# hkchengrex/Cutie

Measured on NVIDIA H100. Metric: frames/sec @480p 3-obj, higher is better.
Workload: dtype f32

## Files before the change

cutie_b200/csrc/conv_tc.cu:

```cuda
#include "common.cuh"
#include "tc_ptx.cuh"

namespace cutie {

namespace {

constexpr int CV_M = 128;
constexpr int CV_KC = 32;
constexpr int CV_A_STAGES = 3;
constexpr int CV_THREADS = 384;
constexpr int CV_WARPS = CV_THREADS / 32;
constexpr int CV_PROD = 128;
constexpr int CV3_ROWS = 248;
constexpr int CV1_ROWS = 128;
constexpr int CV_STAGING = 65 * 1024;

__host__ __device__ constexpr int cv_row_bytes(bool f16) { return f16 ? 64 : 128; }
__host__ __device__ constexpr int cv_planes(bool f16) { return f16 ? 1 : 2; }
__host__ __device__ constexpr int cv_a_bytes(bool f16) { return cv_planes(f16) * CV_M * cv_row_bytes(f16); }
__host__ __device__ constexpr int cv_x_bytes(int ks, bool f16) {
  const int operands = (ks == 3 ? 2 * CV3_ROWS : 4 * CV1_ROWS) * cv_planes(f16) * cv_row_bytes(f16);
  return operands > CV_STAGING ? operands : CV_STAGING;
}

struct ConvTail {
  unsigned long long a_full[2][CV_A_STAGES], a_empty[2][CV_A_STAGES], x_full[4], x_empty[4];
  int last[2];
};
constexpr int cv_smem(int ks, bool f16) { return cv_x_bytes(ks, f16) + CV_A_STAGES * cv_a_bytes(f16) + (int)sizeof(ConvTail) + 64; }

struct ConvTcParams {
  const float* x;
  const unsigned char* wimg;
  const float* bias;
  const float* z;
  float* y;
  long long xs_n, xs_c, xs_p;
  long long ys_n, ys_c, ys_p;
  long long zs_n, zs_c, zs_p;
  int Cin, Cout, H, W;
  int Hi, Wi, stride;
  int TH, TW, tiles_x;
  int pitch, xoff;
  int plane_rows;
  int shift[9];
  int N;
  int relu_in, relu_out, x_vec;
  int cl_vec;
  int q;
  int T, tiles, cots;
  int maxslots;
  float* ws;
  int* counters;
};

struct ConvPart {
  int tile, cot, nb;
  int ty0, tx0;
  long long pix0;
  int c0, c1;
  int slot, nslots;
  long long tile_lin;
};

template <int KS, bool F16>
__global__ void __launch_bounds__(CV_THREADS, 1) conv_tc_kernel(const ConvTcParams p) {
  constexpr int XROWS = KS == 3 ? CV3_ROWS : CV1_ROWS;
  constexpr int ROWB = cv_row_bytes(F16);
  constexpr int XPLANE = XROWS * ROWB;
  constexpr int XSTAGE = cv_planes(F16) * XPLANE;
  constexpr int XST = KS == 3 ? 2 : 4;
  constexpr int A_BYTES = cv_a_bytes(F16);
  constexpr int TAPS = KS * KS;
  constexpr int RPT = KS == 3 ? 2 : 1;
  constexpr int DEPTH = KS == 3 ? 1 : 2;
  constexpr int A_HALF = 64 * ROWB;
  extern __shared__ __align__(1024) unsigned char smem[];
  unsigned char* Xs = smem;
  unsigned char* As = smem + cv_x_bytes(KS, F16);
  ConvTail& T = *reinterpret_cast<ConvTail*>(As + CV_A_STAGES * A_BYTES);
  const int tid = threadIdx.x, lane = tid & 31, warp = tid >> 5;
  const int TWp = p.pitch;
  const int C = p.Cin / CV_KC;
  const long long HW = (long long)p.H * p.W;
  const long long U = (long long)p.T * C;
  const long long u0 = (long long)blockIdx.x * p.q, u1 = u0 + p.q < U ? u0 + p.q : U;
  auto make_part = [&](long long ua, long long ub) {
    ConvPart P;
    P.tile_lin = ua / C;
    P.c0 = (int)(ua - P.tile_lin * C);
    P.c1 = P.c0 + (int)(ub - ua);
    const long long first = (P.tile_lin * C) / p.q, last = (P.tile_lin * C + C - 1) / p.q;
    P.slot = (int)(blockIdx.x - first);
    P.nslots = (int)(last - first + 1);
    P.tile = (int)(P.tile_lin % p.tiles);
    const long long rest = P.tile_lin / p.tiles;
    P.cot = (int)(rest % p.cots);
    P.nb = (int)(rest / p.cots);
    P.ty0 = KS == 3 ? (P.tile / p.tiles_x) * p.TH : 0;
    P.tx0 = KS == 3 ? (P.tile % p.tiles_x) * p.TW : 0;
    P.pix0 = (long long)P.tile * p.N;
    return P;
  };
  const long long split_at = (u0 / C + 1) * C < u1 ? (u0 / C + 1) * C : u1;
  const int nparts = split_at < u1 ? 2 : 1;
  const ConvPart part0 = make_part(u0, split_at), part1 = make_part(nparts == 2 ? split_at : u0, u1);
  const bool direct = nparts == 1 && part0.nslots == 1;

  if (tid == 0) {
    for (int G = 0; G < 2; ++G)
      for (int s = 0; s < CV_A_STAGES; ++s) { mbar_init(smem_u32(&T.a_full[G][s]), 1); mbar_init(smem_u32(&T.a_empty[G][s]), 128); }
    for (int s = 0; s < XST; ++s) { mbar_init(smem_u32(&T.x_full[s]), CV_PROD); mbar_init(smem_u32(&T.x_empty[s]), 256); }
    T.last[0] = T.last[1] = 0;
    mbar_init_fence();
  }
  __syncthreads();
  const bool staged_nchw = p.ys_p == 1 && (p.z == nullptr || p.zs_p == 1);
  const bool staged = staged_nchw || p.cl_vec;
  const int LD = p.N | 1;
  auto store_staged_rows = [&](const ConvPart& P, int sw) {
    const float* stage = reinterpret_cast<const float*>(smem);
    if (!staged_nchw) {
      const int co4 = P.cot * CV_M + 4 * lane;
      if (co4 >= p.Cout) return;
      const float4 b4 = p.bias ? __ldg(reinterpret_cast<const float4*>(p.bias + co4)) : make_float4(0.f, 0.f, 0.f, 0.f);
      for (int j = sw; j < p.N; j += CV_WARPS) {
        long long pix;
        bool ok;
        if (KS == 3) {
          const int ty = j / TWp, lx = j - ty * TWp;
          const int gy = P.ty0 + ty, gx = P.tx0 + lx - p.xoff;
          ok = lx >= p.xoff && lx < p.TW + p.xoff && ty < p.TH && gy < p.H && gx < p.W;
          pix = (long long)gy * p.W + gx;
        } else {
          pix = P.pix0 + j;
          ok = pix < HW;
        }
        if (!ok) continue;
        float4 v = *reinterpret_cast<const float4*>(stage + j * CV_M + 4 * lane);
        v.x += b4.x; v.y += b4.y; v.z += b4.z; v.w += b4.w;
        if (p.z) {
          const float4 z4 = __ldg(reinterpret_cast<const float4*>(p.z + (long long)P.nb * p.zs_n + pix * p.zs_p + co4));
          v.x += z4.x; v.y += z4.y; v.z += z4.z; v.w += z4.w;
        }
        if (p.relu_out) v = make_float4(fmaxf(v.x, 0.f), fmaxf(v.y, 0.f), fmaxf(v.z, 0.f), fmaxf(v.w, 0.f));
        *reinterpret_cast<float4*>(p.y + (long long)P.nb * p.ys_n + pix * p.ys_p + co4) = v;
      }
      return;
    }
    const int nseg = CV_M * (KS == 3 ? p.TH : 1);
    for (int seg = sw; seg < nseg; seg += CV_WARPS) {
      const int col = KS == 3 ? seg / p.TH : seg, ty = KS == 3 ? seg - col * p.TH : 0;
      const int co = P.cot * CV_M + col;
      if (co >= p.Cout) continue;
      long long pbase;
      int len, sbase;
      if (KS == 3) {
        const int gy = P.ty0 + ty;
        if (gy >= p.H) continue;
        pbase = (long long)gy * p.W + P.tx0;
        len = p.W - P.tx0 < p.TW ? p.W - P.tx0 : p.TW;
        sbase = col * LD + ty * TWp + p.xoff;
      } else {
        pbase = P.pix0;
        len = HW - P.pix0 < p.N ? (int)(HW - P.pix0) : p.N;
        sbase = col * LD;
      }
      const float b = p.bias ? __ldg(p.bias + co) : 0.f;
      float* yrow = p.y + (long long)P.nb * p.ys_n + (long long)co * p.ys_c + pbase;
      const float* zrow = p.z ? p.z + (long long)P.nb * p.zs_n + (long long)co * p.zs_c + pbase : nullptr;
      for (int i = lane; i < len; i += 32) {
        float val = stage[sbase + i] + b;
        if (zrow) val += __ldg(zrow + i);
        if (p.relu_out) val = fmaxf(val, 0.f);
        yrow[i] = val;
      }
    }
  };

  auto reduce_shares = [&](const ConvPart& P, int sw, bool to_stage) {
    const int co4 = P.cot * CV_M + 4 * lane;
    const float* wst = p.ws + (P.tile_lin * p.maxslots) * (long long)(p.N * CV_M) + 4 * lane;
    float* stage = reinterpret_cast<float*>(smem);
    const bool co_ok = co4 < p.Cout;
    const float4 b4 = (!to_stage && p.bias && co_ok) ? __ldg(reinterpret_cast<const float4*>(p.bias + co4)) : make_float4(0.f, 0.f, 0.f, 0.f);
    for (int j = sw; j < p.N; j += CV_WARPS) {
      long long pix = 0;
      bool ok = true;
      if (!to_stage) {
        if (KS == 3) {
          const int ty = j / TWp, lx = j - ty * TWp;
          const int gy = P.ty0 + ty, gx = P.tx0 + lx - p.xoff;
          ok = lx >= p.xoff && lx < p.TW + p.xoff && ty < p.TH && gy < p.H && gx < p.W;
          pix = (long long)gy * p.W + gx;
        } else {
          pix = P.pix0 + j;
          ok = pix < HW;
        }
        if (!ok || !co_ok) continue;
      }
      float4 v = __ldcg(reinterpret_cast<const float4*>(wst + (long long)j * CV_M));
      for (int k = 1; k < P.nslots; ++k) {
        const float4 t = __ldcg(reinterpret_cast<const float4*>(wst + ((long long)k * p.N + j) * CV_M));
        v.x += t.x; v.y += t.y; v.z += t.z; v.w += t.w;
      }
      if (to_stage) {
        stage[(4 * lane + 0) * LD + j] = v.x; stage[(4 * lane + 1) * LD + j] = v.y;
        stage[(4 * lane + 2) * LD + j] = v.z; stage[(4 * lane + 3) * LD + j] = v.w;
      } else {
        v.x += b4.x; v.y += b4.y; v.z += b4.z; v.w += b4.w;
        if (p.z) {
          const float4 z4 = __ldg(reinterpret_cast<const float4*>(p.z + (long long)P.nb * p.zs_n + pix * p.zs_p + co4));
          v.x += z4.x; v.y += z4.y; v.z += z4.z; v.w += z4.w;
        }
        if (p.relu_out) v = make_float4(fmaxf(v.x, 0.f), fmaxf(v.y, 0.f), fmaxf(v.z, 0.f), fmaxf(v.w, 0.f));
        *reinterpret_cast<float4*>(p.y + (long long)P.nb * p.ys_n + pix * p.ys_p + co4) = v;
      }
    }
  };

  if (warp >= 8) {
    const int pt = tid - 256;
    int xc = 0;
    for (int pi = 0; pi < nparts; ++pi) {
      const ConvPart& P = pi ? part1 : part0;
      const int chunks = P.c1 - P.c0;
      bool valid[RPT];
      const float* xb[RPT];
#pragma unroll
      for (int h = 0; h < RPT; ++h) {
        const int r = pt + CV_PROD * h;
        bool ok = false;
        long long poff = 0;
        if (KS == 3) {
          if (p.stride == 1) {
            const int rows_used = p.N + 2 * TWp + 2;
            if (r >= 1 && r < rows_used) {
              const int q = r - 1, ly = q / TWp, lx = q - ly * TWp;
              const int gy = P.ty0 + ly - 1, gx = P.tx0 + lx - 1;
              ok = ly < p.TH + 2 && gy >= 0 && gy < p.Hi && gx >= 0 && gx < p.Wi;
              poff = (long long)gy * p.Wi + gx;
            }
          } else {
            const int pl = r / p.plane_rows, q = r - pl * p.plane_rows;
            const int lu = q / TWp, lv = q - lu * TWp;
            const int gy = 2 * (P.ty0 - 1 + lu) + (pl >> 1), gx = 2 * (P.tx0 - 1 + lv) + (pl & 1);
            ok = pl < 4 && lu <= p.TH && gy >= 0 && gy < p.Hi && gx >= 0 && gx < p.Wi;
            poff = (long long)gy * p.Wi + gx;
          }
        } else {
          const long long op = P.pix0 + r;
          if (r < p.N && op < HW) {
            const int oy = (int)(op / p.W), ox = (int)(op - (long long)oy * p.W);
            ok = true;
            poff = (long long)(oy * p.stride) * p.Wi + ox * p.stride;
          }
        }
        valid[h] = ok;
        xb[h] = p.x + (long long)P.nb * p.xs_n + poff * p.xs_p + (long long)(P.c0 * CV_KC) * p.xs_c;
      }
      float v[DEPTH][RPT][CV_KC];
      auto load = [&](int c, float (&dst)[RPT][CV_KC]) {
#pragma unroll
        for (int h = 0; h < RPT; ++h) {
          if (p.x_vec) {
#pragma unroll
            for (int k4 = 0; k4 < CV_KC / 4; ++k4) {
              const float4 f = valid[h] ? __ldg(reinterpret_cast<const float4*>(xb[h] + c * CV_KC + 4 * k4)) : make_float4(0.f, 0.f, 0.f, 0.f);
              dst[h][4 * k4] = f.x; dst[h][4 * k4 + 1] = f.y; dst[h][4 * k4 + 2] = f.z; dst[h][4 * k4 + 3] = f.w;
            }
          } else {
#pragma unroll
            for (int i = 0; i < CV_KC; ++i) dst[h][i] = valid[h] ? __ldg(xb[h] + (long long)(c * CV_KC + i) * p.xs_c) : 0.f;
          }
        }
      };
#pragma unroll
      for (int d = 0; d < DEPTH; ++d)
        if (d < chunks) load(d, v[d]);
#pragma unroll 1
      for (int cb = 0; cb < chunks; cb += DEPTH) {
#pragma unroll
        for (int d = 0; d < DEPTH; ++d) {
          const int c = cb + d;
          if (c < chunks) {
            const int s = xc % XST;
            mbar_wait(smem_u32(&T.x_empty[s]), ((xc / XST) & 1) ^ 1);
#pragma unroll
            for (int rh = 0; rh < RPT; ++rh) {
              const int r = pt + CV_PROD * rh;
              if (r >= XROWS) continue;
              const float* src = v[d][rh];
              if (F16) {
                unsigned char* row = Xs + s * XSTAGE + r * ROWB;
#pragma unroll
                for (int k8 = 0; k8 < CV_KC / 8; ++k8) {
                  float f[8];
#pragma unroll
                  for (int i = 0; i < 8; ++i) f[i] = p.relu_in ? fmaxf(src[8 * k8 + i], 0.f) : src[8 * k8 + i];
                  const int off = (k8 ^ ((r >> 1) & 3)) << 4;
                  *reinterpret_cast<uint4*>(row + off) =
                      make_uint4(f16x2_rn(f[0], f[1]), f16x2_rn(f[2], f[3]), f16x2_rn(f[4], f[5]), f16x2_rn(f[6], f[7]));
                }
              } else {
                unsigned char* hi = Xs + s * XSTAGE + r * 128;
                unsigned char* lo = hi + XPLANE;
#pragma unroll
                for (int k4 = 0; k4 < CV_KC / 4; ++k4) {
                  float4 f = make_float4(src[4 * k4], src[4 * k4 + 1], src[4 * k4 + 2], src[4 * k4 + 3]);
                  if (p.relu_in) f = make_float4(fmaxf(f.x, 0.f), fmaxf(f.y, 0.f), fmaxf(f.z, 0.f), fmaxf(f.w, 0.f));
                  const float4 h = make_float4(to_tf32(f.x), to_tf32(f.y), to_tf32(f.z), to_tf32(f.w));
                  const float4 l = make_float4(to_tf32(f.x - h.x), to_tf32(f.y - h.y), to_tf32(f.z - h.z), to_tf32(f.w - h.w));
                  const int off = (k4 ^ (r & 7)) << 4;
                  *reinterpret_cast<float4*>(hi + off) = h;
                  *reinterpret_cast<float4*>(lo + off) = l;
                }
              }
            }
            fence_proxy_async();
            mbar_arrive(smem_u32(&T.x_full[s]));
            ++xc;
            if (c + DEPTH < chunks) load(c + DEPTH, v[d]);
          }
        }
      }
    }
  } else {
    const int G = warp >> 2, g = lane >> 2, t4 = lane & 3;
    const int cbase = 64 * G + 16 * (warp & 3) + g;
    int i = 0, xc = 0;
    const int steps0 = (part0.c1 - part0.c0) * TAPS;
    const int nsteps = steps0 + (nparts == 2 ? (part1.c1 - part1.c0) * TAPS : 0);
    const bool issuer = (tid & 127) == 0;
    const int wstep0 = (part0.cot * C + part0.c0) * TAPS, wstep1 = (part1.cot * C + part1.c0) * TAPS - steps0;
    auto issue_weights = [&](int j) {
      const unsigned char* src = p.wimg + (size_t)((j < steps0 ? wstep0 : wstep1) + j) * A_BYTES + G * A_HALF;
      const int s = j % CV_A_STAGES;
      const uint32_t dst = smem_u32(As + s * A_BYTES) + G * A_HALF, bar = smem_u32(&T.a_full[G][s]);
      mbar_arrive_expect_tx(bar, cv_planes(F16) * A_HALF);
#pragma unroll
      for (int pl = 0; pl < cv_planes(F16); ++pl) bulk_g2s(dst + pl * CV_M * ROWB, src + pl * CV_M * ROWB, A_HALF, bar);
    };
    if (issuer)
      for (int j = 0; j < CV_A_STAGES && j < nsteps; ++j) issue_weights(j);
    for (int pi = 0; pi < nparts; ++pi) {
      const ConvPart& P = pi ? part1 : part0;
      const int chunks = P.c1 - P.c0;
      float d[64], tot[64];
#pragma unroll
      for (int k = 0; k < 64; ++k) tot[k] = 0.f;
      wg_fence_acc(d);
      for (int c = 0; c < chunks; ++c, ++xc) {
        const int xs = xc % XST;
        mbar_wait(smem_u32(&T.x_full[xs]), (xc / XST) & 1);
        const uint32_t xb_hi = smem_u32(Xs + xs * XSTAGE), xb_lo = xb_hi + XPLANE;
#pragma unroll 1
        for (int t = 0; t < TAPS; ++t, ++i) {
          const int s = i % CV_A_STAGES;
          mbar_wait(smem_u32(&T.a_full[G][s]), (i / CV_A_STAGES) & 1);
          const uint32_t a_hi = smem_u32(As + s * A_BYTES) + G * 64 * ROWB, a_lo = a_hi + CV_M * 128;
          const uint32_t shift = KS == 3 ? (uint32_t)p.shift[t] * ROWB : 0u;
          wg_fence();
          if constexpr (F16) {
#pragma unroll
            for (int ks = 0; ks < 2; ++ks)
              wgmma_f16_n128(d, desc_sw64_kmajor(a_hi + ks * 32), desc_sw64_kmajor(xb_hi + shift + ks * 32), ks);
          } else {
#pragma unroll
            for (int ks = 0; ks < 4; ++ks) {
              const uint64_t da_hi = desc_sw128_kmajor(a_hi + ks * 32), da_lo = desc_sw128_kmajor(a_lo + ks * 32);
              const uint64_t db_hi = desc_sw128_kmajor(xb_hi + shift + ks * 32);
              const uint64_t db_lo = desc_sw128_kmajor(xb_lo + shift + ks * 32);
              wgmma_tf32_n128(d, da_lo, db_hi, ks != 0 ? 1 : 0);
              wgmma_tf32_n128(d, da_hi, db_lo, 1);
              wgmma_tf32_n128(d, da_hi, db_hi, 1);
            }
          }
          wg_commit();
          wg_wait0();
          wg_fence_acc(d);
          mbar_arrive(smem_u32(&T.a_empty[G][s]));
          if (issuer && i + CV_A_STAGES < nsteps) {
            mbar_wait(smem_u32(&T.a_empty[G][s]), (i / CV_A_STAGES) & 1);
            issue_weights(i + CV_A_STAGES);
          }
#pragma unroll
          for (int k = 0; k < 64; ++k) tot[k] += d[k];
        }
        mbar_arrive(smem_u32(&T.x_empty[xs]));
      }
      if (direct) {
        const bool to_stage = staged;
        if (to_stage) asm volatile("bar.sync 1, 256;" ::: "memory");
        float* stage = reinterpret_cast<float*>(smem);
#pragma unroll
        for (int k = 0; k < 64; ++k) {
          const int col = cbase + 8 * ((k >> 1) & 1), pos = 8 * (k >> 2) + 2 * t4 + (k & 1);
          if (pos >= p.N) continue;
          if (to_stage) {
            if (staged_nchw) stage[col * LD + pos] = tot[k];
            else stage[pos * CV_M + col] = tot[k];
            continue;
          }
          const int co = P.cot * CV_M + col;
          bool ok;
          long long pix;
          if (KS == 3) {
            const int ty = pos / TWp, lx = pos - ty * TWp;
            const int gy = P.ty0 + ty, gx = P.tx0 + lx - p.xoff;
            ok = lx >= p.xoff && lx < p.TW + p.xoff && ty < p.TH && gy < p.H && gx < p.W;
            pix = (long long)gy * p.W + gx;
          } else {
            pix = P.pix0 + pos;
            ok = pix < HW;
          }
          if (co < p.Cout && ok) {
            float val = tot[k] + (p.bias ? __ldg(p.bias + co) : 0.f);
            if (p.z) val += __ldg(p.z + (long long)P.nb * p.zs_n + (long long)co * p.zs_c + pix * p.zs_p);
            if (p.relu_out) val = fmaxf(val, 0.f);
            p.y[(long long)P.nb * p.ys_n + (long long)co * p.ys_c + pix * p.ys_p] = val;
          }
        }
        if (tid == 0) T.last[0] = 1;
      } else {
        float* mine = p.ws + (P.tile_lin * p.maxslots + P.slot) * (long long)(p.N * CV_M);
#pragma unroll
        for (int k = 0; k < 64; ++k) {
          const int col = cbase + 8 * ((k >> 1) & 1), pos = 8 * (k >> 2) + 2 * t4 + (k & 1);
          if (pos < p.N) mine[pos * CV_M + col] = tot[k];
        }
      }
    }
    if (!direct) {
      __threadfence();
      asm volatile("bar.sync 1, 256;" ::: "memory");
      if (tid < nparts) {
        const ConvPart& P = tid ? part1 : part0;
        T.last[tid] = atomicAdd(p.counters + P.tile_lin, 1) == P.nslots - 1 ? 1 : 0;
      }
    }
  }
  for (int pi = 0; pi < nparts; ++pi) {
    const ConvPart& P = pi ? part1 : part0;
    asm volatile("bar.sync 2, 384;" ::: "memory");
    const bool fin = T.last[pi] != 0;
    if (!direct && fin) {
      __threadfence();
      if (staged_nchw) {
        reduce_shares(P, warp, true);
      } else if (p.cl_vec) {
        reduce_shares(P, warp, false);
      } else if (warp < 4) {
        const float* wst = p.ws + (P.tile_lin * p.maxslots) * (long long)(p.N * CV_M);
        const int co = P.cot * CV_M + tid;
        const float b = (p.bias && co < p.Cout) ? __ldg(p.bias + co) : 0.f;
        float* yb = p.y + (long long)P.nb * p.ys_n + (long long)co * p.ys_c;
        const float* zb = p.z ? p.z + (long long)P.nb * p.zs_n + (long long)co * p.zs_c : nullptr;
        for (int j = 0; j < p.N; ++j) {
          bool ok;
          long long pix;
          if (KS == 3) {
            const int ty = j / TWp, lx = j - ty * TWp;
            const int gy = P.ty0 + ty, gx = P.tx0 + lx - p.xoff;
            ok = lx >= p.xoff && lx < p.TW + p.xoff && ty < p.TH && gy < p.H && gx < p.W;
            pix = (long long)gy * p.W + gx;
          } else {
            pix = P.pix0 + j;
            ok = pix < HW;
          }
          if (!ok || co >= p.Cout) continue;
          float val = 0.f;
          for (int k = 0; k < P.nslots; ++k) val += __ldcg(wst + ((long long)k * p.N + j) * CV_M + tid);
          val += b;
          if (zb) val += __ldg(zb + pix * p.zs_p);
          if (p.relu_out) val = fmaxf(val, 0.f);
          yb[pix * p.ys_p] = val;
        }
      }
    }
    if (staged_nchw) {
      if (!direct) asm volatile("bar.sync 2, 384;" ::: "memory");
      if (fin) store_staged_rows(P, warp);
    } else if (direct && p.cl_vec) {
      store_staged_rows(P, warp);
    }
    if (pi + 1 < nparts) asm volatile("bar.sync 2, 384;" ::: "memory");
    if (!direct && fin && tid == 0) p.counters[P.tile_lin] = 0;
  }
}

__global__ void __launch_bounds__(256) conv_weight_image_kernel(const float* __restrict__ w, int Cout, int Cin, int taps,
                                                                unsigned char* __restrict__ img) {
  const int chunks = Cin / CV_KC;
  const long long total = (long long)((Cout + CV_M - 1) / CV_M * CV_M) * chunks * taps * 8;
  const long long f = (long long)blockIdx.x * 256 + threadIdx.x;
  if (f >= total) return;
  const int k4 = (int)(f & 7);
  long long g = f >> 3;
  const int row = (int)(g % CV_M); g /= CV_M;
  const int t = (int)(g % taps); g /= taps;
  const int c = (int)(g % chunks);
  const int cot = (int)(g / chunks);
  const int co = cot * CV_M + row;
  float v[4];
#pragma unroll
  for (int i = 0; i < 4; ++i) v[i] = co < Cout ? w[((long long)co * Cin + c * CV_KC + 4 * k4 + i) * taps + t] : 0.f;
  const float4 h = make_float4(to_tf32(v[0]), to_tf32(v[1]), to_tf32(v[2]), to_tf32(v[3]));
  const float4 l = make_float4(to_tf32(v[0] - h.x), to_tf32(v[1] - h.y), to_tf32(v[2] - h.z), to_tf32(v[3] - h.w));
  unsigned char* blk = img + (((size_t)cot * chunks + c) * taps + t) * cv_a_bytes(false);
  const int off = row * 128 + ((k4 ^ (row & 7)) << 4);
  *reinterpret_cast<float4*>(blk + off) = h;
  *reinterpret_cast<float4*>(blk + CV_M * 128 + off) = l;
}

__global__ void __launch_bounds__(256) conv_weight_image_f16_kernel(const float* __restrict__ w, int Cout, int Cin, int taps,
                                                                    unsigned char* __restrict__ img) {
  const int chunks = Cin / CV_KC;
  const long long total = (long long)((Cout + CV_M - 1) / CV_M * CV_M) * chunks * taps * 4;
  const long long f = (long long)blockIdx.x * 256 + threadIdx.x;
  if (f >= total) return;
  const int k8 = (int)(f & 3);
  long long g = f >> 2;
  const int row = (int)(g % CV_M); g /= CV_M;
  const int t = (int)(g % taps); g /= taps;
  const int c = (int)(g % chunks);
  const int cot = (int)(g / chunks);
  const int co = cot * CV_M + row;
  float v[8];
#pragma unroll
  for (int i = 0; i < 8; ++i) v[i] = co < Cout ? w[((long long)co * Cin + c * CV_KC + 8 * k8 + i) * taps + t] : 0.f;
  unsigned char* blk = img + (((size_t)cot * chunks + c) * taps + t) * cv_a_bytes(true);
  *reinterpret_cast<uint4*>(blk + row * 64 + ((k8 ^ ((row >> 1) & 3)) << 4)) =
      make_uint4(f16x2_rn(v[0], v[1]), f16x2_rn(v[2], v[3]), f16x2_rn(v[4], v[5]), f16x2_rn(v[6], v[7]));
}

}

}

using namespace cutie;

#define CONV_REQUIRE(cond, what)                                                          \
  do {                                                                                    \
    if (!(cond)) return ::cutie::fail(-1, "%s: invalid argument: " what, fn);            \
  } while (0)

static int64_t conv_weight_image_bytes(int64_t Cout, int64_t Cin, int ksize, bool f16) {
  if (Cout < 1 || Cin < CV_KC || Cin % CV_KC || (ksize != 1 && ksize != 3)) return -1;
  return ((Cout + CV_M - 1) / CV_M) * (Cin / CV_KC) * ksize * ksize * (int64_t)cv_a_bytes(f16);
}

static int conv_weight_image(const char* fn, bool f16, const float* weight, int64_t Cout, int64_t Cin, int ksize, void* image,
                             void* stream) {
  CONV_REQUIRE(weight && image, "null argument");
  CONV_REQUIRE(ksize == 1 || ksize == 3, "1x1 or 3x3");
  CONV_REQUIRE(Cout >= 1 && Cin >= CV_KC && Cin % CV_KC == 0, "input channels must be a multiple of 32");
  const int taps = ksize * ksize;
  const long long pieces = (Cout + CV_M - 1) / CV_M * CV_M * (Cin / CV_KC) * taps;
  if (f16)
    conv_weight_image_f16_kernel<<<(unsigned)((pieces * 4 + 255) / 256), 256, 0, (cudaStream_t)stream>>>(
        weight, (int)Cout, (int)Cin, taps, static_cast<unsigned char*>(image));
  else
    conv_weight_image_kernel<<<(unsigned)((pieces * 8 + 255) / 256), 256, 0, (cudaStream_t)stream>>>(
        weight, (int)Cout, (int)Cin, taps, static_cast<unsigned char*>(image));
  const cudaError_t e = cudaGetLastError();
  return e == cudaSuccess ? 0 : ::cutie::set_cuda_error(fn, e);
}

extern "C" int64_t cutie_conv_weight_image_bytes(int64_t Cout, int64_t Cin, int ksize) {
  return conv_weight_image_bytes(Cout, Cin, ksize, false);
}

extern "C" int cutie_conv_weight_image(const float* weight, int64_t Cout, int64_t Cin, int ksize, void* image, void* stream) {
  return conv_weight_image(__func__, false, weight, Cout, Cin, ksize, image, stream);
}

extern "C" int64_t cutie_conv_weight_image_f16_bytes(int64_t Cout, int64_t Cin, int ksize) {
  return conv_weight_image_bytes(Cout, Cin, ksize, true);
}

extern "C" int cutie_conv_weight_image_f16(const float* weight, int64_t Cout, int64_t Cin, int ksize, void* image, void* stream) {
  return conv_weight_image(__func__, true, weight, Cout, Cin, ksize, image, stream);
}

static int conv_plane_rows(int th, int tw, int n) { return (th + 1) * (tw + 1) + (n - th * (tw + 1)) + 1; }
static void conv_tile_shape(int H, int W, int stride, int* TH, int* TW, int* N) {
  double best = -1;
  const int pad = stride == 1 ? 2 : 1;
  for (int parts = 1; parts <= W; ++parts) {
    const int tw = (W + parts - 1) / parts;
    for (int th = 1; th <= H && th * (tw + pad) <= 128; ++th) {
      const int n = (th * (tw + pad) + 15) / 16 * 16;
      if (stride == 1 ? n + 2 * (tw + 2) + 2 > CV3_ROWS : 4 * conv_plane_rows(th, tw, n) > CV3_ROWS) continue;
      const long long tiles = (long long)((H + th - 1) / th) * ((W + tw - 1) / tw);
      const double eff = (double)H * W / ((double)tiles * n);
      if (eff > best + 1e-9 || (eff > best - 1e-9 && n > *N)) { best = eff; *TH = th; *TW = tw; *N = n; }
    }
    if (tw <= 8) break;
  }
}

struct ConvPlan { long long tiles, cots, T; int N, C, q, maxslots; long long ctas; int th, tw; };
static int conv_make_plan(int64_t NB, int64_t Cin, int64_t Cout, int64_t H_in, int64_t W_in, int ksize, int stride, int q_override,
                          ConvPlan* pl) {
  const int H = (int)((H_in - 1) / stride + 1), W = (int)((W_in - 1) / stride + 1);
  pl->th = pl->tw = 0; pl->N = 0;
  if (ksize == 3) {
    conv_tile_shape(H, W, stride, &pl->th, &pl->tw, &pl->N);
    if (pl->N < 16) return -1;
    pl->tiles = (long long)((W + pl->tw - 1) / pl->tw) * ((H + pl->th - 1) / pl->th);
  } else {
    const long long hw = (long long)H * W;
    pl->N = hw >= 128 ? 128 : (int)((hw + 15) / 16 * 16);
    pl->tiles = (hw + pl->N - 1) / pl->N;
  }
  pl->cots = (Cout + CV_M - 1) / CV_M;
  pl->T = pl->tiles * pl->cots * NB;
  pl->C = (int)(Cin / CV_KC);
  int q = pl->C;
  for (int s = 2; s <= 8; ++s)
    if (pl->C % s == 0 && pl->T * s <= num_sms() && pl->C / s >= 2) q = pl->C / s;
  if (q_override > 0) q = q_override < pl->C ? q_override : pl->C;
  pl->q = q;
  pl->maxslots = (pl->C - 1) / q + 2;
  pl->ctas = (pl->T * pl->C + q - 1) / q;
  return 0;
}

extern "C" int cutie_conv_plan(int64_t NB, int64_t Cin, int64_t Cout, int64_t H_in, int64_t W_in, int ksize, int stride,
                               int units_per_cta, int64_t* out6) {
  CUTIE_REQUIRE(out6 && (ksize == 1 || ksize == 3) && (stride == 1 || stride == 2) && Cin >= CV_KC && Cin % CV_KC == 0 && NB >= 1 &&
                    Cout >= 1, "bad arguments");
  ConvPlan pl;
  CUTIE_REQUIRE(conv_make_plan(NB, Cin, Cout, H_in, W_in, ksize, stride, units_per_cta, &pl) == 0, "no tile shape for this geometry");
  out6[0] = pl.T; out6[1] = pl.N; out6[2] = pl.C; out6[3] = pl.q; out6[4] = pl.ctas;
  out6[5] = pl.q < pl.C ? pl.T * pl.maxslots * (long long)pl.N * CV_M : 0;
  return 0;
}

template <bool F16>
static int conv_tc_launch(const char* fn, const float* x, const int64_t* x_strides, const void* weight_image, const float* bias,
                          const float* residual, const int64_t* residual_strides, int64_t NB, int64_t Cin, int64_t Cout,
                          int64_t H_in, int64_t W_in, int ksize, int stride, int relu_in, int relu_out, float* y,
                          const int64_t* y_strides, int units_per_cta, float* workspace, int32_t* counters, void* stream) {
  CONV_REQUIRE(x && x_strides && weight_image && y && y_strides, "null argument");
  CONV_REQUIRE(residual == nullptr || residual_strides != nullptr, "residual needs strides");
  CONV_REQUIRE((ksize == 3 || ksize == 1) && (stride == 1 || stride == 2), "3x3 (zero pad 1) or 1x1, stride 1 or 2");
  CONV_REQUIRE(Cout >= 1 && Cin >= CV_KC && Cin % CV_KC == 0, "input channels must be a multiple of 32");
  CONV_REQUIRE(NB >= 1 && NB <= 65535 && H_in >= 1 && W_in >= 1 && H_in * W_in < (1ll << 30), "bad geometry");
  ConvPlan pl;
  CONV_REQUIRE(conv_make_plan(NB, Cin, Cout, H_in, W_in, ksize, stride, units_per_cta, &pl) == 0, "no tile shape for this geometry");
  CONV_REQUIRE(pl.q == pl.C || (workspace && counters), "shared tiles need the workspace and zeroed counters (cutie_conv_plan)");
  CONV_REQUIRE(pl.ctas <= 0x7fffffff, "too many tiles");
  ConvTcParams p;
  p.x = x; p.wimg = static_cast<const unsigned char*>(weight_image); p.bias = bias; p.z = residual; p.y = y;
  p.xs_n = x_strides[0]; p.xs_c = x_strides[1]; p.xs_p = x_strides[2];
  p.ys_n = y_strides[0]; p.ys_c = y_strides[1]; p.ys_p = y_strides[2];
  p.zs_n = residual ? residual_strides[0] : 0;
  p.zs_c = residual ? residual_strides[1] : 0;
  p.zs_p = residual ? residual_strides[2] : 0;
  p.Cin = (int)Cin; p.Cout = (int)Cout; p.Hi = (int)H_in; p.Wi = (int)W_in; p.stride = stride;
  p.H = (int)((H_in - 1) / stride + 1); p.W = (int)((W_in - 1) / stride + 1);
  p.relu_in = relu_in; p.relu_out = relu_out;
  p.x_vec = (p.xs_c == 1 && p.xs_p % 4 == 0 && p.xs_n % 4 == 0 && reinterpret_cast<uintptr_t>(x) % 16 == 0) ? 1 : 0;
  auto vec4 = [](const void* ptr, long long sn, long long sc, long long sp) {
    return sc == 1 && sp % 4 == 0 && sn % 4 == 0 && reinterpret_cast<uintptr_t>(ptr) % 16 == 0;
  };
  p.cl_vec = (Cout % 4 == 0 && vec4(y, p.ys_n, p.ys_c, p.ys_p) && (bias == nullptr || reinterpret_cast<uintptr_t>(bias) % 16 == 0) &&
              (residual == nullptr || vec4(residual, p.zs_n, p.zs_c, p.zs_p))) ? 1 : 0;
  p.TH = pl.th; p.TW = pl.tw; p.N = pl.N; p.tiles_x = 1; p.pitch = 2; p.xoff = 0; p.plane_rows = 0;
  for (int t = 0; t < 9; ++t) p.shift[t] = 0;
  if (ksize == 3) {
    p.tiles_x = (p.W + p.TW - 1) / p.TW;
    if (stride == 1) {
      p.pitch = p.TW + 2; p.xoff = 1;
      for (int t = 0; t < 9; ++t) p.shift[t] = (t / 3) * p.pitch + (t % 3);
    } else {
      p.pitch = p.TW + 1; p.xoff = 0; p.plane_rows = conv_plane_rows(p.TH, p.TW, p.N);
      for (int t = 0; t < 9; ++t) {
        const int dy = t / 3, dx = t % 3;
        const int plane = (dy != 1 ? 2 : 0) + (dx != 1 ? 1 : 0);
        p.shift[t] = plane * p.plane_rows + (dy == 0 ? 0 : 1) * p.pitch + (dx == 0 ? 0 : 1);
      }
    }
  }
  p.q = pl.q; p.T = (int)pl.T; p.tiles = (int)pl.tiles; p.cots = (int)pl.cots; p.maxslots = pl.maxslots;
  p.ws = workspace; p.counters = counters;
  CONV_REQUIRE(pl.T <= 0x7fffffff, "too many tiles");
  static bool attr_done[64] = {};
  if (first_use_on_device(attr_done)) {
    cudaFuncSetAttribute(conv_tc_kernel<3, F16>, cudaFuncAttributeMaxDynamicSharedMemorySize, cv_smem(3, F16));
    cudaFuncSetAttribute(conv_tc_kernel<1, F16>, cudaFuncAttributeMaxDynamicSharedMemorySize, cv_smem(1, F16));
  }
  if (ksize == 3)
    conv_tc_kernel<3, F16><<<(unsigned)pl.ctas, CV_THREADS, cv_smem(3, F16), (cudaStream_t)stream>>>(p);
  else
    conv_tc_kernel<1, F16><<<(unsigned)pl.ctas, CV_THREADS, cv_smem(1, F16), (cudaStream_t)stream>>>(p);
  const cudaError_t e = cudaGetLastError();
  return e == cudaSuccess ? 0 : ::cutie::set_cuda_error(fn, e);
}

extern "C" int cutie_conv_tc(const float* x, const int64_t* x_strides, const void* weight_image, const float* bias,
                             const float* residual, const int64_t* residual_strides, int64_t NB, int64_t Cin, int64_t Cout,
                             int64_t H_in, int64_t W_in, int ksize, int stride, int relu_in, int relu_out, float* y,
                             const int64_t* y_strides, int units_per_cta, float* workspace, int32_t* counters, void* stream) {
  return conv_tc_launch<false>(__func__, x, x_strides, weight_image, bias, residual, residual_strides, NB, Cin, Cout, H_in, W_in,
                               ksize, stride, relu_in, relu_out, y, y_strides, units_per_cta, workspace, counters, stream);
}

extern "C" int cutie_conv_tc_f16(const float* x, const int64_t* x_strides, const void* weight_image, const float* bias,
                                 const float* residual, const int64_t* residual_strides, int64_t NB, int64_t Cin, int64_t Cout,
                                 int64_t H_in, int64_t W_in, int ksize, int stride, int relu_in, int relu_out, float* y,
                                 const int64_t* y_strides, int units_per_cta, float* workspace, int32_t* counters, void* stream) {
  return conv_tc_launch<true>(__func__, x, x_strides, weight_image, bias, residual, residual_strides, NB, Cin, Cout, H_in, W_in,
                              ksize, stride, relu_in, relu_out, y, y_strides, units_per_cta, workspace, counters, stream);
}

extern "C" int cutie_debug_conv_tile_shape(int64_t H, int64_t W, int* out3) {
  int th = 0, tw = 0, n = 0;
  conv_tile_shape((int)H, (int)W, 1, &th, &tw, &n);
  out3[0] = th; out3[1] = tw; out3[2] = n;
  return 0;
}
```

Before: 109.4.

## Overlap weight refill with MMA and batch epilogue loads for latency hiding

Within the MMA loop, the refill of the previous weight stage and the wait for the next A stage now run while the current wgmma group is still in flight, instead of after it retires. The epilogue, staged-store and split-K reduction loops are rewritten to issue batches of residual and workspace loads before consuming them, which raises memory-level parallelism. Optional clock64 timing stamps are added behind a compile-time flag and compile out by default. The batched loops use more registers, and the reordered barrier waits could change how the stages interleave.

```diff
diff --git a/cutie_b200/csrc/conv_tc.cu b/cutie_b200/csrc/conv_tc.cu
--- a/cutie_b200/csrc/conv_tc.cu
+++ b/cutie_b200/csrc/conv_tc.cu
@@ -14,6 +14,7 @@
 constexpr int CV3_ROWS = 248;
 constexpr int CV1_ROWS = 128;
 constexpr int CV_STAGING = 65 * 1024;
+constexpr int EPI_BATCH = 4;
 
 __host__ __device__ constexpr int cv_row_bytes(bool f16) { return f16 ? 64 : 128; }
 __host__ __device__ constexpr int cv_planes(bool f16) { return f16 ? 1 : 2; }
@@ -28,6 +29,46 @@
   int last[2];
 };
 constexpr int cv_smem(int ks, bool f16) { return cv_x_bytes(ks, f16) + CV_A_STAGES * cv_a_bytes(f16) + (int)sizeof(ConvTail) + 64; }
+
+enum StampSlot {
+  ST_STEPS,
+  ST_XFULL,
+  ST_AFULL,
+  ST_MMA,
+  ST_REFILL,
+  ST_PROMOTE,
+  ST_PROLOGUE,
+  ST_EPILOGUE,
+  ST_N
+};
+#ifdef CUTIE_CONV_STAMPS
+constexpr int CV_STAMP_CTAS = 64;
+__device__ unsigned int g_conv_stamps[CV_STAMP_CTAS][2][ST_N];
+struct StepStamps {
+  unsigned long long t0 = 0, last = 0;
+  unsigned int acc[ST_N] = {};
+  __device__ __forceinline__ unsigned long long now() const { return clock64(); }
+  __device__ __forceinline__ void add(int slot, unsigned long long since) { acc[slot] += (unsigned int)(clock64() - since); }
+  __device__ __forceinline__ void step() { acc[ST_STEPS] += 1; last = clock64(); }
+  template <int NR>
+  __device__ __forceinline__ void order(float (&v)[NR]) { wg_fence_acc(v); }
+  __device__ __forceinline__ void write(int G) {
+    if (blockIdx.x >= CV_STAMP_CTAS) return;
+    add(ST_EPILOGUE, last);
+    for (int s = 0; s < ST_N; ++s) g_conv_stamps[blockIdx.x][G][s] = acc[s];
+  }
+};
+#else
+struct StepStamps {
+  unsigned long long t0 = 0;
+  __device__ __forceinline__ unsigned long long now() const { return 0; }
+  __device__ __forceinline__ void add(int, unsigned long long) {}
+  __device__ __forceinline__ void step() {}
+  template <int NR>
+  __device__ __forceinline__ void order(float (&)[NR]) {}
+  __device__ __forceinline__ void write(int) {}
+};
+#endif
 
 struct ConvTcParams {
   const float* x;
@@ -75,6 +116,8 @@
   constexpr int RPT = KS == 3 ? 2 : 1;
   constexpr int DEPTH = KS == 3 ? 1 : 2;
   constexpr int A_HALF = 64 * ROWB;
+  StepStamps stamps;
+  stamps.t0 = stamps.now();
   extern __shared__ __align__(1024) unsigned char smem[];
   unsigned char* Xs = smem;
   unsigned char* As = smem + cv_x_bytes(KS, F16);
@@ -124,56 +167,76 @@
       const int co4 = P.cot * CV_M + 4 * lane;
       if (co4 >= p.Cout) return;
       const float4 b4 = p.bias ? __ldg(reinterpret_cast<const float4*>(p.bias + co4)) : make_float4(0.f, 0.f, 0.f, 0.f);
-      for (int j = sw; j < p.N; j += CV_WARPS) {
-        long long pix;
-        bool ok;
+      for (int j0 = sw; j0 < p.N; j0 += EPI_BATCH * CV_WARPS) {
+        long long pix[EPI_BATCH];
+        bool ok[EPI_BATCH];
+        float4 z4[EPI_BATCH];
+#pragma unroll
+        for (int h = 0; h < EPI_BATCH; ++h) {
+          const int j = j0 + h * CV_WARPS;
+          if (KS == 3) {
+            const int ty = j / TWp, lx = j - ty * TWp;
+            const int gy = P.ty0 + ty, gx = P.tx0 + lx - p.xoff;
+            ok[h] = j < p.N && lx >= p.xoff && lx < p.TW + p.xoff && ty < p.TH && gy < p.H && gx < p.W;
+            pix[h] = (long long)gy * p.W + gx;
+          } else {
+            pix[h] = P.pix0 + j;
+            ok[h] = j < p.N && pix[h] < HW;
+          }
+          z4[h] = p.z && ok[h] ? __ldg(reinterpret_cast<const float4*>(p.z + (long long)P.nb * p.zs_n + pix[h] * p.zs_p + co4))
+                               : make_float4(0.f, 0.f, 0.f, 0.f);
+        }
+#pragma unroll
+        for (int h = 0; h < EPI_BATCH; ++h) {
+          if (!ok[h]) continue;
+          float4 v = *reinterpret_cast<const float4*>(stage + (j0 + h * CV_WARPS) * CV_M + 4 * lane);
+          v.x += b4.x; v.y += b4.y; v.z += b4.z; v.w += b4.w;
+          if (p.z) { v.x += z4[h].x; v.y += z4[h].y; v.z += z4[h].z; v.w += z4[h].w; }
+          if (p.relu_out) v = make_float4(fmaxf(v.x, 0.f), fmaxf(v.y, 0.f), fmaxf(v.z, 0.f), fmaxf(v.w, 0.f));
+          *reinterpret_cast<float4*>(p.y + (long long)P.nb * p.ys_n + pix[h] * p.ys_p + co4) = v;
+        }
+      }
+      return;
+    }
+    const int nseg = CV_M * (KS == 3 ? p.TH : 1);
+    for (int seg0 = sw; seg0 < nseg; seg0 += EPI_BATCH * CV_WARPS) {
+      int len[EPI_BATCH], sbase[EPI_BATCH];
+      float b[EPI_BATCH], zv[EPI_BATCH][4];
+      float* yrow[EPI_BATCH];
+#pragma unroll
+      for (int h = 0; h < EPI_BATCH; ++h) {
+        const int seg = seg0 + h * CV_WARPS;
+        const int col = KS == 3 ? seg / p.TH : seg, ty = KS == 3 ? seg - col * p.TH : 0;
+        const int co = P.cot * CV_M + col;
+        long long pbase;
+        len[h] = 0;
         if (KS == 3) {
-          const int ty = j / TWp, lx = j - ty * TWp;
-          const int gy = P.ty0 + ty, gx = P.tx0 + lx - p.xoff;
-          ok = lx >= p.xoff && lx < p.TW + p.xoff && ty < p.TH && gy < p.H && gx < p.W;
-          pix = (long long)gy * p.W + gx;
+          const int gy = P.ty0 + ty;
+          pbase = (long long)gy * p.W + P.tx0;
+          if (seg < nseg && co < p.Cout && gy < p.H) len[h] = p.W - P.tx0 < p.TW ? p.W - P.tx0 : p.TW;
+          sbase[h] = col * LD + ty * TWp + p.xoff;
         } else {
-          pix = P.pix0 + j;
-          ok = pix < HW;
-        }
-        if (!ok) continue;
-        float4 v = *reinterpret_cast<const float4*>(stage + j * CV_M + 4 * lane);
-        v.x += b4.x; v.y += b4.y; v.z += b4.z; v.w += b4.w;
-        if (p.z) {
-          const float4 z4 = __ldg(reinterpret_cast<const float4*>(p.z + (long long)P.nb * p.zs_n + pix * p.zs_p + co4));
-          v.x += z4.x; v.y += z4.y; v.z += z4.z; v.w += z4.w;
-        }
-        if (p.relu_out) v = make_float4(fmaxf(v.x, 0.f), fmaxf(v.y, 0.f), fmaxf(v.z, 0.f), fmaxf(v.w, 0.f));
-        *reinterpret_cast<float4*>(p.y + (long long)P.nb * p.ys_n + pix * p.ys_p + co4) = v;
-      }
-      return;
-    }
-    const int nseg = CV_M * (KS == 3 ? p.TH : 1);
-    for (int seg = sw; seg < nseg; seg += CV_WARPS) {
-      const int col = KS == 3 ? seg / p.TH : seg, ty = KS == 3 ? seg - col * p.TH : 0;
-      const int co = P.cot * CV_M + col;
-      if (co >= p.Cout) continue;
-      long long pbase;
-      int len, sbase;
-      if (KS == 3) {
-        const int gy = P.ty0 + ty;
-        if (gy >= p.H) continue;
-        pbase = (long long)gy * p.W + P.tx0;
-        len = p.W - P.tx0 < p.TW ? p.W - P.tx0 : p.TW;
-        sbase = col * LD + ty * TWp + p.xoff;
-      } else {
-        pbase = P.pix0;
-        len = HW - P.pix0 < p.N ? (int)(HW - P.pix0) : p.N;
-        sbase = col * LD;
-      }
-      const float b = p.bias ? __ldg(p.bias + co) : 0.f;
-      float* yrow = p.y + (long long)P.nb * p.ys_n + (long long)co * p.ys_c + pbase;
-      const float* zrow = p.z ? p.z + (long long)P.nb * p.zs_n + (long long)co * p.zs_c + pbase : nullptr;
-      for (int i = lane; i < len; i += 32) {
-        float val = stage[sbase + i] + b;
-        if (zrow) val += __ldg(zrow + i);
-        if (p.relu_out) val = fmaxf(val, 0.f);
-        yrow[i] = val;
+          pbase = P.pix0;
+          if (seg < nseg && co < p.Cout) len[h] = HW - P.pix0 < p.N ? (int)(HW - P.pix0) : p.N;
+          sbase[h] = col * LD;
+        }
+        b[h] = p.bias && len[h] ? __ldg(p.bias + co) : 0.f;
+        yrow[h] = p.y + (long long)P.nb * p.ys_n + (long long)co * p.ys_c + pbase;
+        const float* zrow = p.z ? p.z + (long long)P.nb * p.zs_n + (long long)co * p.zs_c + pbase : nullptr;
+#pragma unroll
+        for (int k = 0; k < 4; ++k) zv[h][k] = zrow && lane + 32 * k < len[h] ? __ldg(zrow + lane + 32 * k) : 0.f;
+      }
+#pragma unroll
+      for (int h = 0; h < EPI_BATCH; ++h) {
+#pragma unroll
+        for (int k = 0; k < 4; ++k) {
+          const int i = lane + 32 * k;
+          if (i >= len[h]) continue;
+          float val = stage[sbase[h] + i] + b[h];
+          if (p.z) val += zv[h][k];
+          if (p.relu_out) val = fmaxf(val, 0.f);
+          yrow[h][i] = val;
+        }
       }
     }
   };
@@ -184,37 +247,53 @@
     float* stage = reinterpret_cast<float*>(smem);
     const bool co_ok = co4 < p.Cout;
     const float4 b4 = (!to_stage && p.bias && co_ok) ? __ldg(reinterpret_cast<const float4*>(p.bias + co4)) : make_float4(0.f, 0.f, 0.f, 0.f);
-    for (int j = sw; j < p.N; j += CV_WARPS) {
-      long long pix = 0;
-      bool ok = true;
-      if (!to_stage) {
-        if (KS == 3) {
-          const int ty = j / TWp, lx = j - ty * TWp;
-          const int gy = P.ty0 + ty, gx = P.tx0 + lx - p.xoff;
-          ok = lx >= p.xoff && lx < p.TW + p.xoff && ty < p.TH && gy < p.H && gx < p.W;
-          pix = (long long)gy * p.W + gx;
+    for (int j0 = sw; j0 < p.N; j0 += EPI_BATCH * CV_WARPS) {
+      long long pix[EPI_BATCH];
+      bool ok[EPI_BATCH];
+      float4 v[EPI_BATCH], z4[EPI_BATCH];
+#pragma unroll
+      for (int h = 0; h < EPI_BATCH; ++h) {
+        const int j = j0 + h * CV_WARPS;
+        pix[h] = 0;
+        ok[h] = j < p.N;
+        if (!to_stage) {
+          if (KS == 3) {
+            const int ty = j / TWp, lx = j - ty * TWp;
+            const int gy = P.ty0 + ty, gx = P.tx0 + lx - p.xoff;
+            ok[h] = ok[h] && lx >= p.xoff && lx < p.TW + p.xoff && ty < p.TH && gy < p.H && gx < p.W;
+            pix[h] = (long long)gy * p.W + gx;
+          } else {
+            pix[h] = P.pix0 + j;
+            ok[h] = ok[h] && pix[h] < HW;
+          }
+          ok[h] = ok[h] && co_ok;
+        }
+        const float4 zero = make_float4(0.f, 0.f, 0.f, 0.f);
+        v[h] = ok[h] ? __ldcg(reinterpret_cast<const float4*>(wst + (long long)j * CV_M)) : zero;
+        z4[h] = !to_stage && p.z && ok[h] ? __ldg(reinterpret_cast<const float4*>(p.z + (long long)P.nb * p.zs_n + pix[h] * p.zs_p + co4))
+                                          : zero;
+      }
+#pragma unroll
+      for (int h = 0; h < EPI_BATCH; ++h) {
+        if (!ok[h]) continue;
+        for (int k = 1; k < P.nslots; ++k) {
+          const float4 t = __ldcg(reinterpret_cast<const float4*>(wst + ((long long)k * p.N + j0 + h * CV_WARPS) * CV_M));
+          v[h].x += t.x; v[h].y += t.y; v[h].z += t.z; v[h].w += t.w;
+        }
+      }
+#pragma unroll
+      for (int h = 0; h < EPI_BATCH; ++h) {
+        if (!ok[h]) continue;
+        const int j = j0 + h * CV_WARPS;
+        if (to_stage) {
+          stage[(4 * lane + 0) * LD + j] = v[h].x; stage[(4 * lane + 1) * LD + j] = v[h].y;
+          stage[(4 * lane + 2) * LD + j] = v[h].z; stage[(4 * lane + 3) * LD + j] = v[h].w;
         } else {
-          pix = P.pix0 + j;
-          ok = pix < HW;
-        }
-        if (!ok || !co_ok) continue;
-      }
-      float4 v = __ldcg(reinterpret_cast<const float4*>(wst + (long long)j * CV_M));
-      for (int k = 1; k < P.nslots; ++k) {
-        const float4 t = __ldcg(reinterpret_cast<const float4*>(wst + ((long long)k * p.N + j) * CV_M));
-        v.x += t.x; v.y += t.y; v.z += t.z; v.w += t.w;
-      }
-      if (to_stage) {
-        stage[(4 * lane + 0) * LD + j] = v.x; stage[(4 * lane + 1) * LD + j] = v.y;
-        stage[(4 * lane + 2) * LD + j] = v.z; stage[(4 * lane + 3) * LD + j] = v.w;
-      } else {
-        v.x += b4.x; v.y += b4.y; v.z += b4.z; v.w += b4.w;
-        if (p.z) {
-          const float4 z4 = __ldg(reinterpret_cast<const float4*>(p.z + (long long)P.nb * p.zs_n + pix * p.zs_p + co4));
-          v.x += z4.x; v.y += z4.y; v.z += z4.z; v.w += z4.w;
-        }
-        if (p.relu_out) v = make_float4(fmaxf(v.x, 0.f), fmaxf(v.y, 0.f), fmaxf(v.z, 0.f), fmaxf(v.w, 0.f));
-        *reinterpret_cast<float4*>(p.y + (long long)P.nb * p.ys_n + pix * p.ys_p + co4) = v;
+          v[h].x += b4.x; v[h].y += b4.y; v[h].z += b4.z; v[h].w += b4.w;
+          if (p.z) { v[h].x += z4[h].x; v[h].y += z4[h].y; v[h].z += z4[h].z; v[h].w += z4[h].w; }
+          if (p.relu_out) v[h] = make_float4(fmaxf(v[h].x, 0.f), fmaxf(v[h].y, 0.f), fmaxf(v[h].z, 0.f), fmaxf(v[h].w, 0.f));
+          *reinterpret_cast<float4*>(p.y + (long long)P.nb * p.ys_n + pix[h] * p.ys_p + co4) = v[h];
+        }
       }
     }
   };
@@ -343,6 +422,16 @@
     };
     if (issuer)
       for (int j = 0; j < CV_A_STAGES && j < nsteps; ++j) issue_weights(j);
+    auto wait_x = [&](int xc_) { mbar_wait(smem_u32(&T.x_full[xc_ % XST]), (xc_ / XST) & 1); };
+    auto wait_a = [&](int i_) { mbar_wait(smem_u32(&T.a_full[G][i_ % CV_A_STAGES]), (i_ / CV_A_STAGES) & 1); };
+    {
+      unsigned long long ts = stamps.now();
+      wait_x(0);
+      stamps.add(ST_XFULL, ts);
+      ts = stamps.now();
+      wait_a(0);
+      stamps.add(ST_AFULL, ts);
+    }
     for (int pi = 0; pi < nparts; ++pi) {
       const ConvPart& P = pi ? part1 : part0;
       const int chunks = P.c1 - P.c0;
@@ -352,14 +441,19 @@
       wg_fence_acc(d);
       for (int c = 0; c < chunks; ++c, ++xc) {
         const int xs = xc % XST;
-        mbar_wait(smem_u32(&T.x_full[xs]), (xc / XST) & 1);
+        if (xc > 0) {
+          const unsigned long long ts = stamps.now();
+          wait_x(xc);
+          stamps.add(ST_XFULL, ts);
+        }
         const uint32_t xb_hi = smem_u32(Xs + xs * XSTAGE), xb_lo = xb_hi + XPLANE;
 #pragma unroll 1
         for (int t = 0; t < TAPS; ++t, ++i) {
           const int s = i % CV_A_STAGES;
-          mbar_wait(smem_u32(&T.a_full[G][s]), (i / CV_A_STAGES) & 1);
           const uint32_t a_hi = smem_u32(As + s * A_BYTES) + G * 64 * ROWB, a_lo = a_hi + CV_M * 128;
           const uint32_t shift = KS == 3 ? (uint32_t)p.shift[t] * ROWB : 0u;
+          const unsigned long long t_mma = stamps.now();
+          if (i == 0) stamps.add(ST_PROLOGUE, stamps.t0);
           wg_fence();
           if constexpr (F16) {
 #pragma unroll
@@ -377,15 +471,27 @@
             }
           }
           wg_commit();
+          unsigned long long ts = stamps.now();
+          if (issuer && i > 0 && i - 1 + CV_A_STAGES < nsteps) {
+            mbar_wait(smem_u32(&T.a_empty[G][(i - 1) % CV_A_STAGES]), ((i - 1) / CV_A_STAGES) & 1);
+            issue_weights(i - 1 + CV_A_STAGES);
+          }
+          stamps.add(ST_REFILL, ts);
+          if (i + 1 < nsteps) {
+            ts = stamps.now();
+            wait_a(i + 1);
+            stamps.add(ST_AFULL, ts);
+          }
           wg_wait0();
           wg_fence_acc(d);
+          stamps.add(ST_MMA, t_mma);
           mbar_arrive(smem_u32(&T.a_empty[G][s]));
-          if (issuer && i + CV_A_STAGES < nsteps) {
-            mbar_wait(smem_u32(&T.a_empty[G][s]), (i / CV_A_STAGES) & 1);
-            issue_weights(i + CV_A_STAGES);
-          }
+          ts = stamps.now();
 #pragma unroll
           for (int k = 0; k < 64; ++k) tot[k] += d[k];
+          stamps.order(tot);
+          stamps.add(ST_PROMOTE, ts);
+          stamps.step();
         }
         mbar_arrive(smem_u32(&T.x_empty[xs]));
       }
@@ -393,32 +499,49 @@
         const bool to_stage = staged;
         if (to_stage) asm volatile("bar.sync 1, 256;" ::: "memory");
         float* stage = reinterpret_cast<float*>(smem);
-#pragma unroll
-        for (int k = 0; k < 64; ++k) {
-          const int col = cbase + 8 * ((k >> 1) & 1), pos = 8 * (k >> 2) + 2 * t4 + (k & 1);
-          if (pos >= p.N) continue;
-          if (to_stage) {
+        if (to_stage) {
+#pragma unroll
+          for (int k = 0; k < 64; ++k) {
+            const int col = cbase + 8 * ((k >> 1) & 1), pos = 8 * (k >> 2) + 2 * t4 + (k & 1);
+            if (pos >= p.N) continue;
             if (staged_nchw) stage[col * LD + pos] = tot[k];
             else stage[pos * CV_M + col] = tot[k];
-            continue;
-          }
-          const int co = P.cot * CV_M + col;
-          bool ok;
-          long long pix;
-          if (KS == 3) {
-            const int ty = pos / TWp, lx = pos - ty * TWp;
-            const int gy = P.ty0 + ty, gx = P.tx0 + lx - p.xoff;
-            ok = lx >= p.xoff && lx < p.TW + p.xoff && ty < p.TH && gy < p.H && gx < p.W;
-            pix = (long long)gy * p.W + gx;
-          } else {
-            pix = P.pix0 + pos;
-            ok = pix < HW;
-          }
-          if (co < p.Cout && ok) {
-            float val = tot[k] + (p.bias ? __ldg(p.bias + co) : 0.f);
-            if (p.z) val += __ldg(p.z + (long long)P.nb * p.zs_n + (long long)co * p.zs_c + pix * p.zs_p);
-            if (p.relu_out) val = fmaxf(val, 0.f);
-            p.y[(long long)P.nb * p.ys_n + (long long)co * p.ys_c + pix * p.ys_p] = val;
+          }
+        } else {
+          const int cb = P.cot * CV_M + cbase;
+          const float bias2[2] = {p.bias && cb < p.Cout ? __ldg(p.bias + cb) : 0.f, p.bias && cb + 8 < p.Cout ? __ldg(p.bias + cb + 8) : 0.f};
+#pragma unroll
+          for (int k0 = 0; k0 < 64; k0 += 8) {
+            long long pix[8];
+            bool ok[8];
+            float zv[8];
+#pragma unroll
+            for (int h = 0; h < 8; ++h) {
+              const int k = k0 + h;
+              const int col = cbase + 8 * ((k >> 1) & 1), pos = 8 * (k >> 2) + 2 * t4 + (k & 1);
+              const int co = P.cot * CV_M + col;
+              if (KS == 3) {
+                const int ty = pos / TWp, lx = pos - ty * TWp;
+                const int gy = P.ty0 + ty, gx = P.tx0 + lx - p.xoff;
+                ok[h] = lx >= p.xoff && lx < p.TW + p.xoff && ty < p.TH && gy < p.H && gx < p.W;
+                pix[h] = (long long)gy * p.W + gx;
+              } else {
+                pix[h] = P.pix0 + pos;
+                ok[h] = pix[h] < HW;
+              }
+              ok[h] = ok[h] && pos < p.N && co < p.Cout;
+              zv[h] = p.z && ok[h] ? __ldg(p.z + (long long)P.nb * p.zs_n + (long long)co * p.zs_c + pix[h] * p.zs_p) : 0.f;
+            }
+#pragma unroll
+            for (int h = 0; h < 8; ++h) {
+              if (!ok[h]) continue;
+              const int k = k0 + h;
+              const int co = cb + 8 * ((k >> 1) & 1);
+              float val = tot[k] + bias2[(k >> 1) & 1];
+              if (p.z) val += zv[h];
+              if (p.relu_out) val = fmaxf(val, 0.f);
+              p.y[(long long)P.nb * p.ys_n + (long long)co * p.ys_c + pix[h] * p.ys_p] = val;
+            }
           }
         }
         if (tid == 0) T.last[0] = 1;
@@ -487,6 +610,7 @@
     if (pi + 1 < nparts) asm volatile("bar.sync 2, 384;" ::: "memory");
     if (!direct && fin && tid == 0) p.counters[P.tile_lin] = 0;
   }
+  if (tid < 256 && (tid & 127) == 0) stamps.write(tid >> 7);
 }
 
 __global__ void __launch_bounds__(256) conv_weight_image_kernel(const float* __restrict__ w, int Cout, int Cin, int taps,
@@ -716,6 +840,18 @@
                               ksize, stride, relu_in, relu_out, y, y_strides, units_per_cta, workspace, counters, stream);
 }
 
+#ifdef CUTIE_CONV_STAMPS
+thread_local char cutie::g_last_error[512];
+extern "C" const char* cutie_b200_last_error() { return cutie::g_last_error; }
+
+extern "C" int cutie_conv_stamps(unsigned int* out, int64_t words, int clear) {
+  CUTIE_REQUIRE(out && words == (int64_t)CV_STAMP_CTAS * 2 * ST_N, "stamp buffer size");
+  const cudaError_t e = clear ? cudaMemcpyToSymbol(g_conv_stamps, out, sizeof(g_conv_stamps))
+                              : cudaMemcpyFromSymbol(out, g_conv_stamps, sizeof(g_conv_stamps));
+  return e == cudaSuccess ? 0 : ::cutie::set_cuda_error(__func__, e);
+}
+#endif
+
 extern "C" int cutie_debug_conv_tile_shape(int64_t H, int64_t W, int* out3) {
   int th = 0, tw = 0, n = 0;
   conv_tile_shape((int)H, (int)W, 1, &th, &tw, &n);
```

After: 124.7, median of 6. 13.9% higher.
